# Many98/Crop2Seg

Measured on AMD Instinct MI355X. Metric: train patches/sec (Tx10x128x128) U-TAE, higher is better.
Workload: dtype f32

## Files before the change

### crop2seg_amd/_lib.py

```python
from __future__ import annotations

import ctypes as C
import os
from typing import Optional

HERE = os.path.dirname(os.path.abspath(__file__))
LIB_PATH = os.environ.get("C2S_LIB", os.path.join(HERE, "libc2s_hip.so"))

c_float_p = C.c_void_p
c_int_p = C.c_void_p

PAD_ZEROS, PAD_REFLECT = 0, 1
SRC_F32, SRC_I16, SRC_U16 = 0, 1, 2
NORM_GROUP, NORM_BATCH = 0, 1


class ConvDesc(C.Structure):
    _fields_ = [(n, C.c_int) for n in (
        "N", "C0", "C1", "Hin", "Win", "Cout", "CoutP", "Hout", "Wout", "OutH", "OutW", "KH", "KW", "S",
        "pad_y", "pad_x", "pad_mode", "osy", "osx", "ooy", "oox", "accumulate", "reflect_adjoint")]


class WgradDesc(C.Structure):
    _fields_ = [(n, C.c_int) for n in (
        "N", "C0", "C1", "Hin", "Win", "Cout", "Hout", "Wout", "KH", "KW", "S", "pad_y", "pad_x", "pad_mode",
        "nslices")]


class NormDesc(C.Structure):
    _fields_ = [("N", C.c_int), ("C", C.c_int), ("HW", C.c_int), ("kind", C.c_int), ("groups", C.c_int),
                ("training", C.c_int), ("eps", C.c_float), ("momentum", C.c_float)]


class LtaeDesc(C.Structure):
    _fields_ = [("B", C.c_int), ("T", C.c_int), ("C", C.c_int), ("HW", C.c_int), ("n_head", C.c_int),
                ("d_model", C.c_int), ("eps", C.c_float), ("dropout_p", C.c_float), ("seed", C.c_uint64),
                ("keep", C.c_void_p), ("seed_dev", C.c_void_p), ("keep_bits", C.c_void_p)]


class AggDesc(C.Structure):
    _fields_ = [(n, C.c_int) for n in ("B", "T", "C", "H", "W", "n_head", "h", "w")]


P = C.c_void_p
I = C.c_int
L = C.c_long
F = C.c_float
SZ = C.c_size_t

SIGNATURES = {
    "c2s_abi_version": (I, []),
    "c2s_last_error": (C.c_char_p, []),
    "c2s_init": (I, [I]),
    "c2s_device_cus": (I, []),
    "c2s_pack_weights": (I, [P, P, I, I, I, I, L, L, C.POINTER(I), P]),
    "c2s_pack_job_bytes": (SZ, []),
    "c2s_pack_job_fill": (I, [P, P, P, I, I, I, I, L, L, I, C.POINTER(I), I]),
    "c2s_pack_job_blocks": (I, [I, I, I, I]),
    "c2s_pack_batch": (I, [P, I, I, P]),
    "c2s_conv_igemm": (I, [C.POINTER(ConvDesc), P, P, P, P, P, P, P]),
    "c2s_conv_xpair": (I, [C.POINTER(ConvDesc), P, P, P, P, P, P]),
    "c2s_conv3x3_smallcin_supported": (I, [C.POINTER(ConvDesc)]),
    "c2s_conv3x3_smallcin": (I, [C.POINTER(ConvDesc), P, P, P, P, P, P]),
    "c2s_winograd_packed_floats": (SZ, [I, I]),
    "c2s_pack_weights_winograd": (I, [P, P, I, I, I, L, L, C.POINTER(I), P]),
    "c2s_conv3x3_winograd": (I, [C.POINTER(ConvDesc), P, P, P, P, P, P, P]),
    "c2s_winograd16_packed_floats": (SZ, [I, I]),
    "c2s_pack_weights_winograd16": (I, [P, P, I, I, I, L, L, C.POINTER(I), P]),
    "c2s_conv3x3_winograd16_supported": (I, [C.POINTER(ConvDesc)]),
    "c2s_conv3x3_winograd16": (I, [C.POINTER(ConvDesc), P, P, P, P, P, P, P]),
    "c2s_s2wino_packed_floats": (SZ, [I, I]),
    "c2s_pack_weights_s2wino": (I, [P, P, I, I, I, L, L, C.POINTER(I), P]),
    "c2s_conv4x4s2_winograd_supported": (I, [C.POINTER(ConvDesc)]),
    "c2s_conv4x4s2_winograd": (I, [C.POINTER(ConvDesc), P, P, P, P, P, P]),
    "c2s_s2dgrad_packed_floats": (SZ, [I, I]),
    "c2s_pack_weights_s2dgrad": (I, [P, P, I, I, I, L, L, C.POINTER(I), P]),
    "c2s_conv4x4s2_dgrad_winograd_supported": (I, [C.POINTER(ConvDesc)]),
    "c2s_conv4x4s2_dgrad_winograd": (I, [C.POINTER(ConvDesc), P, P, P, P, P]),
    "c2s_bf16x3_packed_elems": (SZ, [I, I]),
    "c2s_pack_weights_bf16x3": (I, [P, P, P, I, I, I, I, L, L, C.POINTER(I), P]),
    "c2s_conv3x3_bf16x3": (I, [C.POINTER(ConvDesc), P, P, P, P, P, P, P, P]),
    "c2s_bf16x3_set_single_product": (None, [I]),
    "c2s_wgrad_workspace_floats": (SZ, [C.POINTER(WgradDesc)]),
    "c2s_conv_wgrad": (I, [C.POINTER(WgradDesc), P, P, P, P, SZ, P, P]),
    "c2s_wgrad_algorithms": (I, [I, I]),
    "c2s_wgrad_path": (I, [C.POINTER(WgradDesc), C.POINTER(I)]),
    "c2s_wgrad_reduce": (I, [C.POINTER(WgradDesc), P, P, L, L, C.POINTER(I), I, P]),
    "c2s_wgrad_reduce_job_bytes": (SZ, []),
    "c2s_wgrad_reduce_job_blocks": (I, [C.POINTER(WgradDesc)]),
    "c2s_wgrad_reduce_job_fill": (I, [P, C.POINTER(WgradDesc), P, P, L, L, C.POINTER(I), I, I]),
    "c2s_wgrad_reduce_batch": (I, [P, I, I, P]),
    "c2s_dwconv_fwd": (I, [P, P, P, P, I, I, I, I, I, I, I, I, P]),
    "c2s_dwconv_dgrad": (I, [P, P, P, P, I, I, I, I, I, I, I, I, I, P]),
    "c2s_dwconv_wgrad": (I, [P, P, P, P, P, I, I, I, I, I, I, I, I, P]),
    "c2s_norm_workspace_floats": (SZ, [C.POINTER(NormDesc)]),
    "c2s_norm_fwd": (I, [C.POINTER(NormDesc), P, P, P, P, P, P, P, P, P, P, I, P, SZ, P, F, P]),
    "c2s_norm_bwd": (I, [C.POINTER(NormDesc), P, P, P, P, P, I, P, P, P, P, P, SZ, P, P]),
    "c2s_norm_bwd_params": (I, [C.POINTER(NormDesc), P, P, P, P, P, P]),
    "c2s_norm_onepass_sync_bytes": (SZ, [C.POINTER(NormDesc), I]),
    "c2s_norm_fwd_onepass": (I, [C.POINTER(NormDesc), P, P, P, P, P, P, P, P, P, P, I, P, F, P, SZ, P]),
    "c2s_norm_bwd_onepass": (I, [C.POINTER(NormDesc), P, P, P, P, P, I, P, P, P, P, P, SZ, P, P, SZ, P]),
    "c2s_se_workspace_floats": (SZ, [I, I, I]),
    "c2s_channel_bias_add": (I, [P, P, P, I, I, I, P]),
    "c2s_se_fwd": (I, [P, P, P, P, P, P, P, P, I, I, I, F, P, SZ, P]),
    "c2s_se_bwd": (I, [P, P, P, P, P, P, P, P, P, P, I, I, P, I, I, I, P, SZ, P]),
    "c2s_frame_flags": (I, [P, P, I, L, F, P]),
    "c2s_ltae_attn_fwd": (I, [C.POINTER(LtaeDesc)] + [P] * 13 + [P]),
    "c2s_positional_table": (I, [P, P, L, C.c_float, P]),
    "c2s_ltae_fold_fwd": (I, [P] * 9 + [I, I, P]),
    "c2s_ltae_fold_bwd": (I, [P] * 16 + [I, I, I, P, SZ, P]),
    "c2s_ltae_fold_bwd_workspace_floats": (SZ, []),
    "c2s_ltae_pe_table": (I, [I, P, P, F, P, P, P, P, P, I, P]),
    "c2s_ltae_pe_abs_add": (I, [P, P, P, P, P, I, P]),
    "c2s_ltae_pe_abs_bwd": (I, [P, P, P, P, I, P]),
    "c2s_ltae_pe_fwd": (I, [P, P, P, P, P, I, I, I, I, P]),
    "c2s_ltae_pe_gattn": (I, [P, P, P, P, I, I, I, P]),
    "c2s_ltae_pe_bwd": (I, [I] + [P] * 15 + [I, I, I, P]),
    "c2s_ltae_fwd_workspace_floats": (SZ, [C.POINTER(LtaeDesc)]),
    "c2s_ltae_attn_fwd_ws": (I, [C.POINTER(LtaeDesc)] + [P] * 13 + [P, SZ, P]),
    "c2s_ltae_uses_streaming": (I, [C.POINTER(LtaeDesc)]),
    "c2s_ltae_fwd_path": (I, [C.POINTER(LtaeDesc)]),
    "c2s_ltae_attn_optional": (I, [C.POINTER(LtaeDesc)]),
    "c2s_ltae_paths": (I, [C.POINTER(LtaeDesc), I, P, P]),
    "c2s_ltae_bwd_workspace_floats": (SZ, [C.POINTER(LtaeDesc)]),
    "c2s_ltae_attn_bwd": (I, [C.POINTER(LtaeDesc)] + [P] * 22 + [SZ, P]),
    "c2s_dropout_nchw": (I, [P, P, I, I, I, F, C.c_uint64, P, P, P]),
    "c2s_pixel_gn_fwd": (I, [P, P, P, P, P, I, I, I, I, F, P]),
    "c2s_pixel_gn_bwd_workspace_floats": (SZ, [I, I, I]),
    "c2s_pixel_gn_bwd": (I, [P, P, P, P, P, P, P, I, I, I, I, P, SZ, P]),
    "c2s_attn_head_mean": (I, [P, P, I, L, P]),
    "c2s_attn_head_mean_bwd": (I, [P, P, I, L, I, P]),
    "c2s_frame_mean_weights": (I, [P, P, I, I, I, P]),
    "c2s_temporal_aggregate_fwd": (I, [C.POINTER(AggDesc), P, P, P, P, P]),
    "c2s_temporal_aggregate_bwd_workspace_floats": (SZ, [C.POINTER(AggDesc)]),
    "c2s_temporal_aggregate_bwd": (I, [C.POINTER(AggDesc), P, P, P, P, P, I, P, P, SZ, P]),
    "c2s_cross_entropy_workspace_floats": (SZ, [I, I]),
    "c2s_cross_entropy": (I, [P, P, P, P, P, I, I, I, F, C.c_longlong, P, SZ, P]),
    "c2s_metrics_update": (I, [P, P, P, P, P, P, I, I, I, P]),
    "c2s_confusion_add": (I, [P, P, P, L, I, P]),
    "c2s_loss_meter_add": (I, [P, P, P]),
    "c2s_boundary_target": (I, [P, P, I, I, I, P]),
    "c2s_region_relabel": (I, [P, P, I, I, I, I, C.c_longlong, P]),
    "c2s_focal_ce_workspace_floats": (SZ, []),
    "c2s_focal_ce": (I, [P, P, P, P, I, I, I, F, C.c_longlong, I, P, SZ, P]),
    "c2s_focal_ce_ex": (I, [P, P, P, P, P, I, I, I, F, C.c_longlong, I, I, P, SZ, P]),
    "c2s_smooth_ce_workspace_floats": (SZ, []),
    "c2s_smooth_ce": (I, [P, P, P, P, P, P, I, I, I, I, F, C.c_longlong, I, P, SZ, P]),
    "c2s_smooth_ce_ex": (I, [P, P, P, P, P, P, P, I, I, I, I, F, C.c_longlong, I, I, P, SZ, P]),
    "c2s_parcel_seeds": (I, [P, P, P, P, I, I, I, I, I, I, F, P]),
    "c2s_label_components_workspace_bytes": (SZ, [I, I, I]),
    "c2s_label_components": (I, [P, P, P, I, I, I, I, P, SZ, P, P]),
    "c2s_parcel_vote_workspace_bytes": (SZ, [I, I, I]),
    "c2s_parcel_vote": (I, [P, P, P, P, I, I, I, I, I, F, I, P, SZ, P, P]),
    "c2s_collate_series": (I, [P, I, P, P, P, P, P, I, I, I, I, I, C.POINTER(I), C.POINTER(F), C.POINTER(F), F, P]),
    "c2s_collate_series_ndvi": (I, [P, I, P, P, P, P, P, I, I, I, I, I, C.POINTER(I), C.POINTER(F), C.POINTER(F), F, I, I, P]),
    "c2s_softmax_stitch": (I, [P, P, P, I, I, I, I, I, I, I, I, P]),
    "c2s_adam_flat": (I, [P, P, P, P, L, F, F, F, F, I, P, F, P]),
    "c2s_grad_sumsq_workspace_doubles": (SZ, []),
    "c2s_grad_sumsq": (I, [P, P, P, I, L, P, SZ, P, P]),
    "c2s_step_decide": (I, [P, F, F, I, P, P, I, P, P]),
    "c2s_adam_slots": (I, [P, P, P, P, P, P, P, I, L, F, F, F, F, P, P]),
    "c2s_restore_if_skipped": (I, [P, P, L, P, P]),
    "c2s_fill": (I, [P, L, F, P]),
    "c2s_add_inplace": (I, [P, P, L, P]),
}

_LIB: Optional[C.CDLL] = None


class C2SError(RuntimeError):
    pass


def lib() -> C.CDLL:
    global _LIB
    if _LIB is None:
        if not os.path.exists(LIB_PATH):
            raise C2SError(
                f"{LIB_PATH} not found: build it with `python -m crop2seg_amd.build` "
                "(or __graft_entry__.build()); crop2seg_amd has no CPU/PyTorch fallback")
        handle = C.CDLL(LIB_PATH)
        for name, (res, args) in SIGNATURES.items():
            fn = getattr(handle, name)
            fn.restype = res
            fn.argtypes = args
        _LIB = handle
    return _LIB


_INITED = set()


def init_device(index: int) -> None:
    if index in _INITED:
        return
    check(lib().c2s_init(index), "c2s_init")
    _INITED.add(index)


def check(rc: int, what: str) -> None:
    if rc != 0:
        msg = lib().c2s_last_error().decode(errors="replace")
        raise C2SError(f"{what} failed (code {rc}): {msg}")
```

### crop2seg_amd/csrc/conv_igemm.hip

```cpp
#include "common.h"

namespace {

struct ConvParams {
    const float* src0;
    const float* src1;
    const float* wpk;
    const float* bias;
    float* out;
    const int* valid;
    int C0, C1, Hin, Win, Cout, CoutP, Hout, Wout, OutH, OutW;
    int pad_y, pad_x, pad_mode, osy, osx, ooy, oox, accumulate;
    int log2fc, tiles_x;
    int adj, ay_lo, ay_hi, ax_lo, ax_hi;
    int dy_lo, dy_hi, dx_lo, dx_hi;
};

constexpr int cmax(int a, int b) { return a > b ? a : b; }
constexpr int plane_for(int K, int S, int log2fc) {
    return ((8 * (32 >> log2fc) - 1) * S + K) * (((1 << log2fc) - 1) * S + K);
}
constexpr int max_plane(int K, int S) {
    return cmax(cmax(plane_for(K, S, 2), plane_for(K, S, 3)), cmax(plane_for(K, S, 4), plane_for(K, S, 5)));
}

template <int K, int S>
struct Cfg {
    static constexpr int CK = K == 1 ? 16 : (K == 2 ? 8 : (K >= 4 ? 2 : 4));
    static constexpr int NT = K * K;
    static constexpr int MAXE = (CK * max_plane(K, S) + 255) / 256;
};

template <int K, int S, int MF, bool ADJ>
__global__ __launch_bounds__(256) void conv_igemm_kernel(ConvParams p) {
    constexpr int CK = Cfg<K, S>::CK;
    constexpr int NT = Cfg<K, S>::NT;
    constexpr int MAXE = Cfg<K, S>::MAXE;
    constexpr int COT = 32 * MF;
    constexpr int WV = COT / 4;
    constexpr int NWV = NT * CK * WV;
    constexpr int WPT = (NWV + 255) / 256;
    constexpr int NS = NT * (CK / 2);
    extern __shared__ float lds[];

    int bxi = blockIdx.x, n = blockIdx.z;
    {
        const unsigned tot = gridDim.x * gridDim.z;
        if (gridDim.y == 1 && (tot & 7) == 0) {
            const unsigned lin = blockIdx.x + gridDim.x * blockIdx.z;
            const unsigned l2_ = (lin & 7) * (tot >> 3) + (lin >> 3);
            n = (int)(l2_ / gridDim.x);
            bxi = (int)(l2_ - (unsigned)n * gridDim.x);
        }
    }
    if (p.valid != nullptr && p.valid[n] == 0) return;

    const int FC = 1 << p.log2fc, FR = 32 >> p.log2fc;
    const int tile_h = 8 * FR, tile_w = FC;
    const int rows = (tile_h - 1) * S + K, cols = (tile_w - 1) * S + K;
    const int plane = rows * cols;
    float* Xl = lds;
    const int xsz = (CK * plane + 3) & ~3;
    float* Wl = lds + xsz;
    const int BUF = xsz + NT * CK * COT;

    const int tyi = bxi / p.tiles_x, txi = bxi % p.tiles_x;
    const int oy0 = tyi * tile_h, ox0 = txi * tile_w;
    const int co0 = blockIdx.y * COT;
    const int tid = threadIdx.x;
    const int Cin = p.C0 + p.C1;
    const int HWin = p.Hin * p.Win;

    int goff[MAXE];
    const int total = CK * plane;
#pragma unroll
    for (int i = 0; i < MAXE; ++i) {
        const int e = tid + i * 256;
        int off = -1;
        if (e < total) {
            const int c = e / plane;
            const int rem = e - c * plane;
            const int r = rem / cols;
            const int cc = rem - r * cols;
            int gy = oy0 * S - p.pad_y + r;
            int gx = ox0 * S - p.pad_x + cc;
            bool ok;
            if (p.pad_mode == C2S_PAD_REFLECT) {
                ok = gy >= -p.pad_y && gy < p.Hin + p.pad_y && gx >= -p.pad_x && gx < p.Win + p.pad_x;
                gy = reflect_idx(gy, p.Hin);
                gx = reflect_idx(gx, p.Win);
            } else {
                ok = gy >= 0 && gy < p.Hin && gx >= 0 && gx < p.Win;
            }
            if (ok) off = (c * HWin + gy * p.Win + gx) * 4;
        }
        goff[i] = off;
    }

    const int lane = tid & 63, wave = tid >> 6;
    const int li = lane & 31, lk = lane >> 5;
    const int fy = li >> p.log2fc, fx = li & (FC - 1);
    int boff[2];
#pragma unroll
    for (int q = 0; q < 2; ++q) {
        const int f = 2 * wave + q;
        boff[q] = lk * plane + ((f * FR + fy) * S) * cols + fx * S;
    }
    const int aoff = lk * COT + li;

    float mxlo[2] = {0.f, 0.f}, mxhi[2] = {0.f, 0.f}, mylo[2] = {0.f, 0.f}, myhi[2] = {0.f, 0.f};
    if constexpr (ADJ) {
#pragma unroll
        for (int q = 0; q < 2; ++q) {
            const int f = 2 * wave + q;
            const int oy = oy0 + f * FR + fy, ox = ox0 + fx;
            mxlo[q] = ox == p.ax_lo ? 1.f : 0.f;
            mxhi[q] = ox == p.ax_hi ? 1.f : 0.f;
            mylo[q] = oy == p.ay_lo ? 1.f : 0.f;
            myhi[q] = oy == p.ay_hi ? 1.f : 0.f;
        }
    }

    f32x16 acc[MF][2];
#pragma unroll
    for (int m = 0; m < MF; ++m)
#pragma unroll
        for (int q = 0; q < 2; ++q)
#pragma unroll
            for (int r = 0; r < 16; ++r) acc[m][q][r] = 0.f;

    const float* s0n = p.src0 + (size_t)n * p.C0 * HWin;
    const float* s1n = p.src1 != nullptr ? p.src1 + (size_t)n * p.C1 * HWin : nullptr;
    const __amdgpu_buffer_rsrc_t r0 = __builtin_amdgcn_make_buffer_rsrc((void*)s0n, 0, p.C0 * HWin * 4, 0x00020000);
    const __amdgpu_buffer_rsrc_t r1 = __builtin_amdgcn_make_buffer_rsrc((void*)(s1n != nullptr ? s1n : s0n), 0,
                                                                         p.C1 * HWin * 4, 0x00020000);
    const __amdgpu_buffer_rsrc_t rw = __builtin_amdgcn_make_buffer_rsrc((void*)p.wpk, 0, NT * Cin * p.CoutP * 4, 0x00020000);

    float xr[MAXE];
    f32x4 wr[WPT];
    auto prefetch = [&](int cb) {
        const bool first = cb < p.C0;
        const int chan0 = (first ? cb : cb - p.C0) * HWin * 4;
        if (first) {
#pragma unroll
            for (int i = 0; i < MAXE; ++i)
                xr[i] = __builtin_bit_cast(float, __builtin_amdgcn_raw_buffer_load_b32(r0, goff[i] >= 0 ? goff[i] + chan0 : -1, 0, 0));
        } else {
#pragma unroll
            for (int i = 0; i < MAXE; ++i)
                xr[i] = __builtin_bit_cast(float, __builtin_amdgcn_raw_buffer_load_b32(r1, goff[i] >= 0 ? goff[i] + chan0 : -1, 0, 0));
        }
#pragma unroll
        for (int i = 0; i < WPT; ++i) {
            const int e = tid + i * 256;
            const int o4 = e % WV, tc = e / WV;
            const int c = tc % CK, t = tc / CK;
            const bool ok = e < NWV && cb + c < Cin;
            const int off = ok ? (((t * Cin + cb + c) * p.CoutP + co0 + o4 * 4) * 4) : -1;
            wr[i] = __builtin_bit_cast(f32x4, __builtin_amdgcn_raw_buffer_load_b128(rw, off, 0, 0));
        }
    };
    auto commit = [&](int buf) {
        float* Xd = Xl + buf * BUF;
        float* Wd = Wl + buf * BUF;
#pragma unroll
        for (int i = 0; i < MAXE; ++i) {
            const int e = tid + i * 256;
            if (e < total) Xd[e] = xr[i];
        }
#pragma unroll
        for (int i = 0; i < WPT; ++i) {
            const int e = tid + i * 256;
            if (e < NWV) *reinterpret_cast<f32x4*>(Wd + (size_t)e * 4) = wr[i];
        }
    };

    auto load_ops = [&](const float* Xl, const float* Wl, int s_, float (&a)[MF], float (&b)[2]) {
        const int t = s_ / (CK / 2), cp = s_ % (CK / 2);
        const int ky = t / K, kx = t % K;
#pragma unroll
        for (int m = 0; m < MF; ++m) a[m] = Wl[(t * CK + 2 * cp) * COT + aoff + m * 32];
#pragma unroll
        for (int q = 0; q < 2; ++q) {
            const int ad = boff[q] + 2 * cp * plane + ky * cols + kx;
            float v = Xl[ad];
            if constexpr (ADJ) {
                const bool xl = kx == K - 1, xh = kx == 0, yl = ky == K - 1, yh = ky == 0;
                const int dx = xl ? -p.dx_lo : p.dx_hi;
                if (xl || xh) {
                    const float mx = xl ? mxlo[q] : mxhi[q];
                    v = fmaf(mx, Xl[ad + dx], v);
                }
                if (yl || yh) {
                    const float my = yl ? mylo[q] : myhi[q];
                    const int dy = (yl ? -p.dy_lo : p.dy_hi) * cols;
                    v = fmaf(my, Xl[ad + dy], v);
                    if (xl || xh) {
                        const float mx = xl ? mxlo[q] : mxhi[q];
                        v = fmaf(my * mx, Xl[ad + dy + dx], v);
                    }
                }
            }
            b[q] = v;
        }
    };

    constexpr int COMMIT_AT = NS / 2;
    prefetch(0);
    commit(0);
    if (CK < Cin) prefetch(CK);
    __syncthreads();
    int cur = 0;
    for (int cb = 0; cb < Cin; cb += CK, cur ^= 1) {
        const float* Xc = Xl + cur * BUF;
        const float* Wc = Wl + cur * BUF;
        float a[2][MF], b[2][2];
        load_ops(Xc, Wc, 0, a[0], b[0]);
#pragma unroll
        for (int s_ = 0; s_ < NS; ++s_) {
            if (s_ + 1 < NS) load_ops(Xc, Wc, s_ + 1, a[(s_ + 1) & 1], b[(s_ + 1) & 1]);
            __builtin_amdgcn_sched_barrier(0);
#pragma unroll
            for (int m = 0; m < MF; ++m)
#pragma unroll
                for (int q = 0; q < 2; ++q)
                    acc[m][q] = __builtin_amdgcn_mfma_f32_32x32x2f32(a[s_ & 1][m], b[s_ & 1][q], acc[m][q], 0, 0, 0);
            __builtin_amdgcn_sched_barrier(0);
            if (s_ == COMMIT_AT && cb + CK < Cin) {
                commit(cur ^ 1);
                if (cb + 2 * CK < Cin) prefetch(cb + 2 * CK);
                __builtin_amdgcn_sched_barrier(0);
            }
        }
        __syncthreads();
    }

    const size_t outHW = (size_t)p.OutH * p.OutW;
    float* on = p.out + (size_t)n * p.Cout * outHW;
#pragma unroll
    for (int q = 0; q < 2; ++q) {
        const int f = 2 * wave + q;
        const int oy = oy0 + f * FR + fy, ox = ox0 + fx;
        if (oy >= p.Hout || ox >= p.Wout) continue;
        const size_t sp = (size_t)(oy * p.osy + p.ooy) * p.OutW + (ox * p.osx + p.oox);
#pragma unroll
        for (int m = 0; m < MF; ++m) {
#pragma unroll
            for (int r0 = 0; r0 < 16; r0 += 8) {
                float old[8];
                if (p.accumulate) {
#pragma unroll
                    for (int u = 0; u < 8; ++u) {
                        const int r = r0 + u;
                        const int co = co0 + m * 32 + (r & 3) + 8 * (r >> 2) + 4 * lk;
                        old[u] = co < p.Cout ? on[(size_t)co * outHW + sp] : 0.f;
                    }
                }
#pragma unroll
                for (int u = 0; u < 8; ++u) {
                    const int r = r0 + u;
                    const int co = co0 + m * 32 + (r & 3) + 8 * (r >> 2) + 4 * lk;
                    if (co < p.Cout) {
                        float v = acc[m][q][r];
                        if (p.bias != nullptr) v += p.bias[co];
                        if (p.accumulate) v += old[u];
                        on[(size_t)co * outHW + sp] = v;
                    }
                }
            }
        }
    }
}

template <int K, int S, int MF, bool ADJ>
int launch_conv(const ConvParams& p, int N, int tiles, hipStream_t st) {
    constexpr int CK = Cfg<K, S>::CK;
    constexpr int NT = Cfg<K, S>::NT;
    const int FC = 1 << p.log2fc, FR = 32 >> p.log2fc;
    const int rows = (8 * FR - 1) * S + K, cols = (FC - 1) * S + K;
    const size_t lds = 2 * ((((size_t)CK * rows * cols + 3) & ~(size_t)3) + (size_t)NT * CK * 32 * MF) * sizeof(float);
    dim3 grid(tiles, p.CoutP / (32 * MF), N);
    hipLaunchKernelGGL((conv_igemm_kernel<K, S, MF, ADJ>), grid, dim3(256), lds, st, p);
    C2S_CHECK_LAUNCH("conv_igemm");
    return C2S_OK;
}

void init_hook() {
#define C2S_RAISE4(K_, S_)                               \
    C2S_RAISE_LDS((conv_igemm_kernel<K_, S_, 1, false>)); \
    C2S_RAISE_LDS((conv_igemm_kernel<K_, S_, 2, false>));
    C2S_RAISE4(3, 1) C2S_RAISE4(1, 1) C2S_RAISE4(2, 1) C2S_RAISE4(4, 2) C2S_RAISE4(2, 2) C2S_RAISE4(6, 2)
#undef C2S_RAISE4
    C2S_RAISE_LDS((conv_igemm_kernel<3, 1, 1, true>));
    C2S_RAISE_LDS((conv_igemm_kernel<3, 1, 2, true>));
    C2S_RAISE_LDS((conv_igemm_kernel<2, 1, 1, true>));
    C2S_RAISE_LDS((conv_igemm_kernel<2, 1, 2, true>));
}
C2sInitRegistrar registrar(init_hook);

}

extern "C" int c2s_conv_igemm(const c2s_conv_desc* d, const float* src0, const float* src1, const float* wpk,
                              const float* bias, float* out, const int* valid, void* stream) {
    C2S_REQUIRE(d && src0 && wpk && out, "conv_igemm: null pointer");
    C2S_REQUIRE(d->N > 0 && d->C0 > 0 && d->C1 >= 0 && (d->C1 == 0 || src1), "conv_igemm: bad channels");
    C2S_REQUIRE(d->CoutP % 32 == 0 && d->CoutP >= d->Cout && d->Cout > 0, "conv_igemm: CoutP must be a multiple of 32");
    C2S_REQUIRE(d->KH == d->KW, "conv_igemm: square kernels only");
    C2S_REQUIRE(d->C1 == 0 || d->C0 % 16 == 0, "conv_igemm: with two sources C0 must be a multiple of 16");
    C2S_REQUIRE((long)(d->C0 > d->C1 ? d->C0 : d->C1) * d->Hin * d->Win * 4 < (1L << 31), "conv_igemm: frame too large");
    C2S_REQUIRE((long)d->Hin * d->Win < (1 << 20), "conv_igemm: input plane too large");
    C2S_REQUIRE(d->Hout > 0 && d->Wout > 0, "conv_igemm: empty output");
    C2S_REQUIRE((d->Hout - 1) * d->osy + d->ooy < d->OutH && (d->Wout - 1) * d->osx + d->oox < d->OutW,
                "conv_igemm: output placement exceeds the output plane");
    if (d->pad_mode == C2S_PAD_REFLECT)
        C2S_REQUIRE(d->pad_y < d->Hin && d->pad_x < d->Win, "conv_igemm: reflect padding needs pad < size");
    ConvParams p;
    p.src0 = src0; p.src1 = src1; p.wpk = wpk; p.bias = bias; p.out = out; p.valid = valid;
    p.C0 = d->C0; p.C1 = d->C1; p.Hin = d->Hin; p.Win = d->Win; p.Cout = d->Cout; p.CoutP = d->CoutP;
    p.Hout = d->Hout; p.Wout = d->Wout; p.OutH = d->OutH; p.OutW = d->OutW;
    p.pad_y = d->pad_y; p.pad_x = d->pad_x; p.pad_mode = d->pad_mode;
    p.osy = d->osy; p.osx = d->osx; p.ooy = d->ooy; p.oox = d->oox; p.accumulate = d->accumulate;
    p.adj = d->reflect_adjoint;
    p.ay_lo = p.ay_hi = p.ax_lo = p.ax_hi = -1;
    p.dy_lo = p.dy_hi = p.dx_lo = p.dx_hi = d->KH - 1;
    if (d->reflect_adjoint == 2) {
        C2S_REQUIRE(d->pad_mode == C2S_PAD_ZEROS && d->S == 1 && d->KH == 3 && d->pad_y == 1 && d->pad_x == 1 &&
                    d->osy == 2 && d->osx == 2 && d->ooy >= 0 && d->ooy <= 1 && d->oox >= 0 && d->oox <= 1 &&
                    d->Hin == d->Hout && d->Win == d->Wout && d->Hin >= 2 && d->Win >= 2,
                    "conv_igemm: reflect_adjoint 2 applies to the parity launches of the 6x6 stride-2 data gradient");
        p.ay_lo = d->ooy == 0 ? 1 : 0;   p.dy_lo = d->ooy == 0 ? 2 : 1;
        p.ay_hi = d->Hout - 1 - d->ooy;  p.dy_hi = d->ooy == 0 ? 1 : 2;
        p.ax_lo = d->oox == 0 ? 1 : 0;   p.dx_lo = d->oox == 0 ? 2 : 1;
        p.ax_hi = d->Wout - 1 - d->oox;  p.dx_hi = d->oox == 0 ? 1 : 2;
    } else if (d->reflect_adjoint) {
        C2S_REQUIRE(d->pad_mode == C2S_PAD_ZEROS && d->S == 1 && (d->KH == 3 || d->KH == 2),
                    "conv_igemm: reflect_adjoint applies to the zero-padded 3x3 / 2x2-parity data-gradient launches");
        C2S_REQUIRE(d->Hin >= 2 && d->Win >= 2 && d->Hin != 3 && d->Win != 3, "conv_igemm: reflect_adjoint needs planes of 2 or >= 4");
        if (d->KH == 3) {
            C2S_REQUIRE(d->pad_y == 1 && d->pad_x == 1 && d->Hin == d->Hout && d->Win == d->Wout, "conv_igemm: bad 3x3 adjoint geometry");
            p.ay_lo = 1; p.ay_hi = d->Hout - 2;
            p.ax_lo = 1; p.ax_hi = d->Wout - 2;
        } else {
            if (d->pad_y == 0) p.ay_lo = 0; else p.ay_hi = d->Hout - 1;
            if (d->pad_x == 0) p.ax_lo = 0; else p.ax_hi = d->Wout - 1;
        }
    }
    int l2 = 5;
    while (l2 > 2 && (1 << l2) > d->Wout) --l2;
    p.log2fc = l2;
    const int FC = 1 << l2, FR = 32 >> l2;
    p.tiles_x = cdiv(d->Wout, FC);
    const int tiles = p.tiles_x * cdiv(d->Hout, 8 * FR);
    hipStream_t st = (hipStream_t)stream;
    const int cus = c2s_cus();
    const bool wide = d->CoutP % 64 == 0 && (long)tiles * d->N * (d->CoutP / 64) >= 2L * cus;
#define C2S_DISPATCH(K_, S_, A_)                                        \
    if (d->KH == K_ && d->S == S_ && (p.adj != 0) == A_)                \
        return wide ? launch_conv<K_, S_, 2, A_>(p, d->N, tiles, st) : launch_conv<K_, S_, 1, A_>(p, d->N, tiles, st);
    C2S_DISPATCH(3, 1, false)
    C2S_DISPATCH(3, 1, true)
    C2S_DISPATCH(1, 1, false)
    C2S_DISPATCH(2, 1, false)
    C2S_DISPATCH(2, 1, true)
    C2S_DISPATCH(4, 2, false)
    C2S_DISPATCH(2, 2, false)
    C2S_DISPATCH(6, 2, false)
#undef C2S_DISPATCH
    c2s_set_error("conv_igemm: unsupported (K=%d,S=%d)", d->KH, d->S);
    return C2S_EINVAL;
}
```

### include/c2s_hip.h

```cpp
#ifndef C2S_HIP_H
#define C2S_HIP_H

#include <stddef.h>
#include <stdint.h>

#ifdef __cplusplus
extern "C" {
#endif

#define C2S_OK 0
#define C2S_EINVAL (-1)
#define C2S_ELAUNCH (-2)
#define C2S_ENOSPACE (-3)

#define C2S_PAD_ZEROS 0
#define C2S_PAD_REFLECT 1

#define C2S_NORM_GROUP 0
#define C2S_NORM_BATCH 1

int c2s_abi_version(void);
const char* c2s_last_error(void);
int c2s_init(int device);
int c2s_device_cus(void);

int c2s_pack_weights(const float* src, float* wpk, int cin, int cout, int coutP, int ntaps,
                     long stride_o, long stride_c, const int* host_tap_off, void* stream);
size_t c2s_pack_job_bytes(void);
int c2s_pack_job_fill(void* host_record, const float* src, float* dst, int cin, int cout, int coutP, int ntaps,
                      long stride_o, long stride_c, int winograd, const int* host_tap_off, int block_start);
int c2s_pack_job_blocks(int cin, int coutP, int ntaps, int winograd);
int c2s_pack_batch(const void* device_table, int njobs, int total_blocks, void* stream);


typedef struct c2s_conv_desc {
    int N, C0, C1;
    int Hin, Win;
    int Cout, CoutP;
    int Hout, Wout;
    int OutH, OutW;
    int KH, KW, S;
    int pad_y, pad_x;
    int pad_mode;
    int osy, osx, ooy, oox;
    int accumulate;
    int reflect_adjoint;
} c2s_conv_desc;

int c2s_conv_igemm(const c2s_conv_desc* d, const float* src0, const float* src1, const float* wpk,
                   const float* bias, float* out, const int* valid, void* stream);

int c2s_conv3x3_smallcin_supported(const c2s_conv_desc* d);
int c2s_conv3x3_smallcin(const c2s_conv_desc* d, const float* src, const float* wpk, const float* bias, float* out,
                         const int* valid, void* stream);

int c2s_conv_xpair(const c2s_conv_desc* d, const float* src, const float* wpk, const float* bias, float* out,
                   const int* valid, void* stream);

size_t c2s_winograd_packed_floats(int cin, int coutP);
int c2s_pack_weights_winograd(const float* src, float* upk, int cin, int cout, int coutP, long stride_o, long stride_c,
                              const int* host_tap_off, void* stream);
int c2s_conv3x3_winograd(const c2s_conv_desc* d, const float* src0, const float* src1, const float* upk,
                         const float* bias, float* out, const int* valid, void* stream);

size_t c2s_winograd16_packed_floats(int cin, int coutP);
int c2s_pack_weights_winograd16(const float* src, float* upk, int cin, int cout, int coutP, long stride_o, long stride_c,
                                const int* host_tap_off, void* stream);
int c2s_conv3x3_winograd16_supported(const c2s_conv_desc* d);
int c2s_conv3x3_winograd16(const c2s_conv_desc* d, const float* src0, const float* src1, const float* upk,
                           const float* bias, float* out, const int* valid, void* stream);

size_t c2s_s2wino_packed_floats(int cin, int coutP);
int c2s_pack_weights_s2wino(const float* src, float* upk, int cin, int cout, int coutP, long stride_o, long stride_c,
                            const int* host_tap_off, void* stream);
int c2s_conv4x4s2_winograd_supported(const c2s_conv_desc* d);
int c2s_conv4x4s2_winograd(const c2s_conv_desc* d, const float* src, const float* upk, const float* bias, float* out,
                           const int* valid, void* stream);

size_t c2s_s2dgrad_packed_floats(int kc, int csP);
int c2s_pack_weights_s2dgrad(const float* src, float* upk, int kc, int cs, int csP, long stride_c, long stride_k,
                             const int* host_tap_off, void* stream);
int c2s_conv4x4s2_dgrad_winograd_supported(const c2s_conv_desc* d);
int c2s_conv4x4s2_dgrad_winograd(const c2s_conv_desc* d, const float* gy, const float* upk, float* gx, const int* valid,
                                 void* stream);

size_t c2s_bf16x3_packed_elems(int cin, int coutP);
int c2s_pack_weights_bf16x3(const float* src, void* whi, void* wlo, int cin, int cout, int coutP, int ntaps,
                            long stride_o, long stride_c, const int* host_tap_off, void* stream);
int c2s_conv3x3_bf16x3(const c2s_conv_desc* d, const float* src0, const float* src1, const void* whi,
                       const void* wlo, const float* bias, float* out, const int* valid, void* stream);
void c2s_bf16x3_set_single_product(int on);

typedef struct c2s_wgrad_desc {
    int N, C0, C1, Hin, Win;
    int Cout;
    int Hout, Wout;
    int KH, KW, S, pad_y, pad_x, pad_mode;
    int nslices;
} c2s_wgrad_desc;

size_t c2s_wgrad_workspace_floats(const c2s_wgrad_desc* d);
int c2s_conv_wgrad(const c2s_wgrad_desc* d, const float* src0, const float* src1, const float* gout,
                   float* slabs, size_t slab_floats, const int* valid, void* stream);
int c2s_wgrad_algorithms(int winograd_3x3, int winograd_4x4s2);
int c2s_wgrad_path(const c2s_wgrad_desc* d, int* family);
int c2s_wgrad_reduce(const c2s_wgrad_desc* d, const float* slabs, float* dst, long stride_o, long stride_c,
                     const int* host_tap_off, int accumulate, void* stream);
size_t c2s_wgrad_reduce_job_bytes(void);
int c2s_wgrad_reduce_job_blocks(const c2s_wgrad_desc* d);
int c2s_wgrad_reduce_job_fill(void* host_record, const c2s_wgrad_desc* d, const float* slabs, float* dst, long stride_o,
                              long stride_c, const int* host_tap_off, int accumulate, int block_start);
int c2s_wgrad_reduce_batch(const void* device_table, int njobs, int total_blocks, void* stream);

int c2s_dwconv_fwd(const float* in, const float* w, float* out, const int* valid, int N, int C, int Hin, int Win,
                   int K, int S, int pad, int pad_mode, void* stream);
int c2s_dwconv_dgrad(const float* gout, const float* w, float* gin, const int* valid, int N, int C, int Hin, int Win,
                     int K, int S, int pad, int pad_mode, int accumulate, void* stream);
int c2s_dwconv_wgrad(const float* in, const float* gout, float* partial, float* gw, const int* valid, int N, int C,
                     int Hin, int Win, int K, int S, int pad, int pad_mode, void* stream);

typedef struct c2s_norm_desc {
    int N, C, HW;
    int kind;
    int groups;
    int training;
    float eps, momentum;
} c2s_norm_desc;

size_t c2s_norm_workspace_floats(const c2s_norm_desc* d);
int c2s_norm_fwd(const c2s_norm_desc* d, const float* x, const float* gamma, const float* beta,
                 float* running_mean, float* running_var, long long* num_batches_tracked, float* group_stats, float* row_ab,
                 const float* residual, float* y, int relu, float* workspace, size_t ws_floats, const int* valid,
                 float pad_value, void* stream);
int c2s_norm_bwd(const c2s_norm_desc* d, const float* x, const float* g, const float* gamma,
                 const float* group_stats, const float* row_ab, int relu, float* gx, float* dgamma,
                 float* dbeta, float* dbias, float* workspace, size_t ws_floats, const int* valid, void* stream);
int c2s_norm_bwd_params(const c2s_norm_desc* d, const float* workspace, float* dgamma, float* dbeta, float* dbias,
                        const int* valid, void* stream);

size_t c2s_norm_onepass_sync_bytes(const c2s_norm_desc* d, int has_valid);
int c2s_norm_fwd_onepass(const c2s_norm_desc* d, const float* x, const float* gamma, const float* beta,
                         float* running_mean, float* running_var, long long* num_batches_tracked, float* group_stats,
                         float* row_ab, const float* residual, float* y, int relu, const int* valid, float pad_value,
                         void* sync, size_t sync_bytes, void* stream);
int c2s_norm_bwd_onepass(const c2s_norm_desc* d, const float* x, const float* g, const float* gamma,
                         const float* group_stats, const float* row_ab, int relu, float* gx, float* dgamma, float* dbeta,
                         float* dbias, float* workspace, size_t ws_floats, const int* valid, void* sync,
                         size_t sync_bytes, void* stream);

size_t c2s_se_workspace_floats(int N, int C, int HW);
int c2s_channel_bias_add(float* x, const float* bias, const int* valid, int N, int C, int HW, void* stream);
int c2s_se_fwd(const float* x, const float* W1, const float* W2, float* pooled, float* hidden, float* scale, float* y,
               const int* valid, int N, int C, int HW, float pad_value, float* workspace, size_t ws_floats, void* stream);
int c2s_se_bwd(const float* x, const float* g, const float* W1, const float* W2, const float* pooled, const float* hidden,
               const float* scale, float* gx, float* gW1, float* gW2, int acc_w1, int acc_w2, const int* valid, int N, int C,
               int HW, float* workspace, size_t ws_floats, void* stream);

int c2s_frame_flags(const float* x, int* valid, int N, long frame_elems, float pad_value, void* stream);

typedef struct c2s_ltae_desc {
    int B, T, C, HW;
    int n_head, d_model;
    float eps;
    float dropout_p;
    uint64_t seed;
    const float* keep;
    const uint64_t* seed_dev;
    uint64_t* keep_bits;
} c2s_ltae_desc;

int c2s_ltae_attn_fwd(const c2s_ltae_desc* d, const float* x, const float* gamma, const float* beta,
                      const float* U, const float* s0, const float* Wc, const float* bc, const float* pe,
                      const int* valid, float* attn, float* attn_pre, float* emb, float* stats, void* stream);
size_t c2s_ltae_fwd_workspace_floats(const c2s_ltae_desc* d);
int c2s_ltae_attn_fwd_ws(const c2s_ltae_desc* d, const float* x, const float* gamma, const float* beta,
                         const float* U, const float* s0, const float* Wc, const float* bc, const float* pe,
                         const int* valid, float* attn, float* attn_pre, float* emb, float* stats,
                         float* workspace, size_t ws_floats, void* stream);
int c2s_ltae_uses_streaming(const c2s_ltae_desc* d);
int c2s_ltae_fwd_path(const c2s_ltae_desc* d);
int c2s_ltae_attn_optional(const c2s_ltae_desc* d);
int c2s_ltae_paths(const c2s_ltae_desc* d, int with_emb, int* fwd, int* bwd);
size_t c2s_ltae_bwd_workspace_floats(const c2s_ltae_desc* d);
int c2s_ltae_attn_bwd(const c2s_ltae_desc* d, const float* x, const float* gamma, const float* beta,
                      const float* U, const float* s0, const float* Wc, const float* bc, const float* pe,
                      const int* valid, const float* attn, const float* attn_pre, const float* stats,
                      const float* g_emb, const float* g_attn, float* gx, float* gU, float* gs0, float* gWc,
                      float* gbc, float* ggamma, float* gbeta, float* workspace, size_t ws_floats, void* stream);

int c2s_positional_table(const long long* dates, float* pe, long n, float period, void* stream);
int c2s_ltae_fold_fwd(const float* Q, const float* Wk, const float* bk, const float* Wc, const float* bc, const float* pe,
                      float* U, float* s0, float* qwk, int BT, int C, void* stream);
int c2s_ltae_fold_bwd(const float* Q, const float* Wk, const float* bk, const float* Wc, const float* bc, const float* pe,
                      const float* qwk, const float* gU, const float* gs0, const float* gWc_attn, const float* gbc_attn,
                      float* gQ, float* gWk, float* gbk, float* gWc, float* gbc, int BT, int C, int acc_mask,
                      float* workspace, size_t ws_floats, void* stream);
size_t c2s_ltae_fold_bwd_workspace_floats(void);

int c2s_ltae_pe_table(int mode, const long long* dates0, const long long* dates1, float period, const float* W, const float* b,
                      float* pe256, float* sin256, int* bad_days, int BT, void* stream);
int c2s_ltae_pe_abs_add(const long long* dates1, const float* W2, const float* b2, float* pe256, int* bad_days, int BT,
                        void* stream);
int c2s_ltae_pe_abs_bwd(const long long* dates1, const float* g_pe, float* gW2, float* gb2, int BT, void* stream);
int c2s_ltae_pe_fwd(const float* qwk, const float* pe256, const float* attn, float* s0, float* emb, int B, int T, int HW,
                    int phase, void* stream);
int c2s_ltae_pe_gattn(const float* g_emb, const float* pe256, const float* g_attn_in, float* g_attn_out, int B, int T, int HW,
                      void* stream);
int c2s_ltae_pe_bwd(int mode, const long long* dates0, const long long* dates1, const float* Q, const float* Wk,
                    const float* qwk, const float* pe256, const float* sin256, const float* attn, const float* g_emb,
                    const float* gs0, float* g_pe, float* gWk, float* gQ, float* gW, float* gb, int B, int T, int HW,
                    void* stream);

int c2s_dropout_nchw(const float* x, float* y, int B, int C, int HW, float p, uint64_t seed, const uint64_t* seed_dev,
                     const float* keep, void* stream);
int c2s_pixel_gn_fwd(const float* x, const float* gamma, const float* beta, float* y, float* stats, int B, int C,
                     int HW, int groups, float eps, void* stream);
size_t c2s_pixel_gn_bwd_workspace_floats(int B, int C, int HW);
int c2s_pixel_gn_bwd(const float* x, const float* gy, const float* gamma, const float* stats, float* gx,
                     float* dgamma, float* dbeta, int B, int C, int HW, int groups, float* workspace,
                     size_t ws_floats, void* stream);

typedef struct c2s_agg_desc {
    int B, T, C, H, W;
    int n_head, h, w;
} c2s_agg_desc;

int c2s_attn_head_mean(const float* attn, float* v, int n_head, long n, void* stream);
int c2s_attn_head_mean_bwd(const float* gv, float* gattn, int n_head, long n, int accumulate, void* stream);
int c2s_frame_mean_weights(const int* valid, float* v, int n_head, int B, int T, void* stream);
int c2s_temporal_aggregate_fwd(const c2s_agg_desc* d, const float* x, const float* attn, const int* valid,
                               float* out, void* stream);
size_t c2s_temporal_aggregate_bwd_workspace_floats(const c2s_agg_desc* d);
int c2s_temporal_aggregate_bwd(const c2s_agg_desc* d, const float* x, const float* attn, const int* valid,
                               const float* gout, float* gx, int gx_accumulate, float* gattn,
                               float* workspace, size_t ws_floats, void* stream);

size_t c2s_cross_entropy_workspace_floats(int B, int HW);
int c2s_cross_entropy(const float* logits, const int64_t* target, const float* class_w, float* loss,
                      float* glogits, int B, int K, int HW, float label_smoothing, long long ignore_index,
                      float* workspace, size_t ws_floats, void* stream);
int c2s_adam_flat(float* p, const float* g, float* m, float* v, long n, float lr, float b1, float b2, float eps,
                  int step, const int* step_dev, float grad_scale, void* stream);

#define C2S_GUARD_STATUS_BYTES 32
size_t c2s_grad_sumsq_workspace_doubles(void);
int c2s_grad_sumsq(const float* g, const long* slots, const int* mask, int nslots, long total, double* workspace,
                   size_t ws_doubles, void* status, void* stream);
int c2s_step_decide(void* status, float max_grad_norm, float grad_scale, int skip_nonfinite, const int* mask,
                    int* slot_steps, int nslots, int* skip_count, void* stream);
int c2s_adam_slots(float* p, const float* g, float* m, float* v, const long* slots, const int* mask,
                   const int* slot_steps, int nslots, long total, float lr, float b1, float b2, float eps,
                   const void* status, void* stream);
int c2s_restore_if_skipped(float* dst, const float* saved, long n, const void* status, void* stream);

int c2s_metrics_update(const float* logits, const long long* target, long long* conf, long long* conf_top2,
                       long long* pred, long long* pred_top2, int B, int K, int HW, void* stream);
int c2s_confusion_add(const long long* pred, const long long* target, long long* conf, long n, int K, void* stream);
int c2s_loss_meter_add(const float* loss, double* acc, void* stream);
int c2s_boundary_target(const long long* y, long long* y_b, int B, int H, int W, void* stream);
int c2s_region_relabel(const long long* y, long long* y_out, int B, int H, int W, int keep_boundary, long long ignore_label,
                       void* stream);
size_t c2s_focal_ce_workspace_floats(void);
int c2s_focal_ce(const float* logits, const long long* target, float* loss, float* glogits, int B, int K, int HW,
                 float gamma, long long ignore_index, int accumulate_loss, float* workspace, size_t ws_floats,
                 void* stream);
int c2s_focal_ce_ex(const float* logits, const long long* target, const float* class_w, float* loss, float* glogits, int B,
                    int K, int HW, float gamma, long long ignore_index, int size_average, int accumulate_loss,
                    float* workspace, size_t ws_floats, void* stream);
size_t c2s_smooth_ce_workspace_floats(void);
int c2s_smooth_ce(const float* logits, const long long* target, const float* class_w, const float* bg_distrib, float* loss,
                  float* glogits, int B, int K, int H, int W, float label_smoothing, long long bg_index, int accumulate_loss,
                  float* workspace, size_t ws_floats, void* stream);
int c2s_smooth_ce_ex(const float* logits, const long long* target, const float* class_w, const float* bg_distrib, float* loss,
                     float* glogits, float* pixel_loss, int B, int K, int H, int W, float label_smoothing, long long bg_index,
                     int reduction, int accumulate_loss, float* workspace, size_t ws_floats, void* stream);

int c2s_parcel_seeds(const float* scores, const float* boundary_scores, unsigned char* mask, long long* t1, int B, int K,
                     int H, int W, int from_logits, int boundary_code, float second_threshold, void* stream);
size_t c2s_label_components_workspace_bytes(int B, int H, int W);
int c2s_label_components(const unsigned char* mask, int* labels, int* count, int B, int H, int W, int min_size,
                         void* workspace, size_t ws_bytes, int* error, void* stream);
size_t c2s_parcel_vote_workspace_bytes(int B, int cap, int K);
int c2s_parcel_vote(const long long* pred, const int* labels, long long* out, int* parcel_class, int B, int H, int W, int K,
                    int cap, float bg_share, int outside, void* workspace, size_t ws_bytes, int* error, void* stream);

#define C2S_SRC_F32 0
#define C2S_SRC_I16 1
#define C2S_SRC_U16 2
int c2s_collate_series(const void* src, int src_dtype, const long long* offsets, const long long* src_dates, float* x,
                       long long* dates, int* valid, int B, int T, int C, int Cs, int HW,
                       const int* host_channel_order, const float* host_mean, const float* host_std, float pad_value,
                       void* stream);
int c2s_collate_series_ndvi(const void* src, int src_dtype, const long long* offsets, const long long* src_dates, float* x,
                            long long* dates, int* valid, int B, int T, int C, int Cs, int HW, const int* host_channel_order,
                            const float* host_mean, const float* host_std, float pad_value, int ndvi_a, int ndvi_b,
                            void* stream);
int c2s_softmax_stitch(const float* logits, float* proba, long long* top1, int first_patch, int npatch, int K, int ph,
                       int pw, int grid_w, int out_h, int out_w, void* stream);

int c2s_fill(float* p, long n, float v, void* stream);
int c2s_add_inplace(float* dst, const float* src, long n, void* stream);

#ifdef __cplusplus
}
#endif
#endif
```

Measured before the change: 369.6.

## Split igemm conv spatial tiles into smaller workgroups when grid underfills CUs

Adds split variants of the implicit-GEMM conv kernel that cover half or a quarter of the spatial tile rows. The SP=4 variant uses 128 threads, and both split variants use one fragment per wave and a deeper operand prefetch. A heuristic picks the split when the default grid would have fewer than two workgroups per CU, and an environment variable can force a choice. The aim is better occupancy on small late-layer convolutions. The cost is more redundant halo loads and weight staging per output, and more kernel instantiations.

```diff
diff --git a/crop2seg_amd/_lib.py b/crop2seg_amd/_lib.py
--- a/crop2seg_amd/_lib.py
+++ b/crop2seg_amd/_lib.py
@@ -59,6 +59,7 @@
     "c2s_pack_job_blocks": (I, [I, I, I, I]),
     "c2s_pack_batch": (I, [P, I, I, P]),
     "c2s_conv_igemm": (I, [C.POINTER(ConvDesc), P, P, P, P, P, P, P]),
+    "c2s_conv_igemm_split": (I, [C.POINTER(ConvDesc), I]),
     "c2s_conv_xpair": (I, [C.POINTER(ConvDesc), P, P, P, P, P, P]),
     "c2s_conv3x3_smallcin_supported": (I, [C.POINTER(ConvDesc)]),
     "c2s_conv3x3_smallcin": (I, [C.POINTER(ConvDesc), P, P, P, P, P, P]),
diff --git a/crop2seg_amd/csrc/conv_igemm.hip b/crop2seg_amd/csrc/conv_igemm.hip
--- a/crop2seg_amd/csrc/conv_igemm.hip
+++ b/crop2seg_amd/csrc/conv_igemm.hip
@@ -17,29 +17,35 @@
 };
 
 constexpr int cmax(int a, int b) { return a > b ? a : b; }
-constexpr int plane_for(int K, int S, int log2fc) {
-    return ((8 * (32 >> log2fc) - 1) * S + K) * (((1 << log2fc) - 1) * S + K);
-}
-constexpr int max_plane(int K, int S) {
-    return cmax(cmax(plane_for(K, S, 2), plane_for(K, S, 3)), cmax(plane_for(K, S, 4), plane_for(K, S, 5)));
-}
-
-template <int K, int S>
+constexpr int plane_for(int K, int S, int log2fc, int NF) {
+    return ((NF * (32 >> log2fc) - 1) * S + K) * (((1 << log2fc) - 1) * S + K);
+}
+constexpr int max_plane(int K, int S, int NF) {
+    return cmax(cmax(plane_for(K, S, 2, NF), plane_for(K, S, 3, NF)), cmax(plane_for(K, S, 4, NF), plane_for(K, S, 5, NF)));
+}
+
+template <int K, int S, int SP = 1>
 struct Cfg {
     static constexpr int CK = K == 1 ? 16 : (K == 2 ? 8 : (K >= 4 ? 2 : 4));
     static constexpr int NT = K * K;
-    static constexpr int MAXE = (CK * max_plane(K, S) + 255) / 256;
+    static constexpr int NTHR = SP == 4 ? 128 : 256;
+    static constexpr int MAXE = (CK * max_plane(K, S, 8 / SP) + NTHR - 1) / NTHR;
 };
 
-template <int K, int S, int MF, bool ADJ>
-__global__ __launch_bounds__(256) void conv_igemm_kernel(ConvParams p) {
-    constexpr int CK = Cfg<K, S>::CK;
-    constexpr int NT = Cfg<K, S>::NT;
-    constexpr int MAXE = Cfg<K, S>::MAXE;
+template <int K, int S, int MF, bool ADJ, int SP = 1>
+__global__ __launch_bounds__((Cfg<K, S, SP>::NTHR)) void conv_igemm_kernel(ConvParams p) {
+    static_assert(SP == 1 || ((SP == 2 || SP == 4) && MF == 1), "the split tiles exist for 32-channel tiles");
+    constexpr int CK = Cfg<K, S, SP>::CK;
+    constexpr int NT = Cfg<K, S, SP>::NT;
+    constexpr int MAXE = Cfg<K, S, SP>::MAXE;
+    constexpr int NTHR = Cfg<K, S, SP>::NTHR;
+    constexpr int NF = 8 / SP;
+    constexpr int NQ = SP == 1 ? 2 : 1;
+    constexpr int LA = SP == 1 ? 1 : 2;
     constexpr int COT = 32 * MF;
     constexpr int WV = COT / 4;
     constexpr int NWV = NT * CK * WV;
-    constexpr int WPT = (NWV + 255) / 256;
+    constexpr int WPT = (NWV + NTHR - 1) / NTHR;
     constexpr int NS = NT * (CK / 2);
     extern __shared__ float lds[];
 
@@ -56,7 +62,7 @@
     if (p.valid != nullptr && p.valid[n] == 0) return;
 
     const int FC = 1 << p.log2fc, FR = 32 >> p.log2fc;
-    const int tile_h = 8 * FR, tile_w = FC;
+    const int tile_h = NF * FR, tile_w = FC;
     const int rows = (tile_h - 1) * S + K, cols = (tile_w - 1) * S + K;
     const int plane = rows * cols;
     float* Xl = lds;
@@ -75,7 +81,7 @@
     const int total = CK * plane;
 #pragma unroll
     for (int i = 0; i < MAXE; ++i) {
-        const int e = tid + i * 256;
+        const int e = tid + i * NTHR;
         int off = -1;
         if (e < total) {
             const int c = e / plane;
@@ -100,19 +106,19 @@
     const int lane = tid & 63, wave = tid >> 6;
     const int li = lane & 31, lk = lane >> 5;
     const int fy = li >> p.log2fc, fx = li & (FC - 1);
-    int boff[2];
-#pragma unroll
-    for (int q = 0; q < 2; ++q) {
-        const int f = 2 * wave + q;
+    int boff[NQ];
+#pragma unroll
+    for (int q = 0; q < NQ; ++q) {
+        const int f = NQ * wave + q;
         boff[q] = lk * plane + ((f * FR + fy) * S) * cols + fx * S;
     }
     const int aoff = lk * COT + li;
 
-    float mxlo[2] = {0.f, 0.f}, mxhi[2] = {0.f, 0.f}, mylo[2] = {0.f, 0.f}, myhi[2] = {0.f, 0.f};
+    float mxlo[NQ] = {}, mxhi[NQ] = {}, mylo[NQ] = {}, myhi[NQ] = {};
     if constexpr (ADJ) {
 #pragma unroll
-        for (int q = 0; q < 2; ++q) {
-            const int f = 2 * wave + q;
+        for (int q = 0; q < NQ; ++q) {
+            const int f = NQ * wave + q;
             const int oy = oy0 + f * FR + fy, ox = ox0 + fx;
             mxlo[q] = ox == p.ax_lo ? 1.f : 0.f;
             mxhi[q] = ox == p.ax_hi ? 1.f : 0.f;
@@ -121,11 +127,11 @@
         }
     }
 
-    f32x16 acc[MF][2];
+    f32x16 acc[MF][NQ];
 #pragma unroll
     for (int m = 0; m < MF; ++m)
 #pragma unroll
-        for (int q = 0; q < 2; ++q)
+        for (int q = 0; q < NQ; ++q)
 #pragma unroll
             for (int r = 0; r < 16; ++r) acc[m][q][r] = 0.f;
 
@@ -152,7 +158,7 @@
         }
 #pragma unroll
         for (int i = 0; i < WPT; ++i) {
-            const int e = tid + i * 256;
+            const int e = tid + i * NTHR;
             const int o4 = e % WV, tc = e / WV;
             const int c = tc % CK, t = tc / CK;
             const bool ok = e < NWV && cb + c < Cin;
@@ -165,23 +171,23 @@
         float* Wd = Wl + buf * BUF;
 #pragma unroll
         for (int i = 0; i < MAXE; ++i) {
-            const int e = tid + i * 256;
+            const int e = tid + i * NTHR;
             if (e < total) Xd[e] = xr[i];
         }
 #pragma unroll
         for (int i = 0; i < WPT; ++i) {
-            const int e = tid + i * 256;
+            const int e = tid + i * NTHR;
             if (e < NWV) *reinterpret_cast<f32x4*>(Wd + (size_t)e * 4) = wr[i];
         }
     };
 
-    auto load_ops = [&](const float* Xl, const float* Wl, int s_, float (&a)[MF], float (&b)[2]) {
+    auto load_ops = [&](const float* Xl, const float* Wl, int s_, float (&a)[MF], float (&b)[NQ]) {
         const int t = s_ / (CK / 2), cp = s_ % (CK / 2);
         const int ky = t / K, kx = t % K;
 #pragma unroll
         for (int m = 0; m < MF; ++m) a[m] = Wl[(t * CK + 2 * cp) * COT + aoff + m * 32];
 #pragma unroll
-        for (int q = 0; q < 2; ++q) {
+        for (int q = 0; q < NQ; ++q) {
             const int ad = boff[q] + 2 * cp * plane + ky * cols + kx;
             float v = Xl[ad];
             if constexpr (ADJ) {
@@ -214,17 +220,18 @@
     for (int cb = 0; cb < Cin; cb += CK, cur ^= 1) {
         const float* Xc = Xl + cur * BUF;
         const float* Wc = Wl + cur * BUF;
-        float a[2][MF], b[2][2];
-        load_ops(Xc, Wc, 0, a[0], b[0]);
+        float a[LA + 1][MF], b[LA + 1][NQ];
+#pragma unroll
+        for (int s_ = 0; s_ < LA; ++s_) load_ops(Xc, Wc, s_, a[s_], b[s_]);
 #pragma unroll
         for (int s_ = 0; s_ < NS; ++s_) {
-            if (s_ + 1 < NS) load_ops(Xc, Wc, s_ + 1, a[(s_ + 1) & 1], b[(s_ + 1) & 1]);
+            if (s_ + LA < NS) load_ops(Xc, Wc, s_ + LA, a[(s_ + LA) % (LA + 1)], b[(s_ + LA) % (LA + 1)]);
             __builtin_amdgcn_sched_barrier(0);
 #pragma unroll
             for (int m = 0; m < MF; ++m)
 #pragma unroll
-                for (int q = 0; q < 2; ++q)
-                    acc[m][q] = __builtin_amdgcn_mfma_f32_32x32x2f32(a[s_ & 1][m], b[s_ & 1][q], acc[m][q], 0, 0, 0);
+                for (int q = 0; q < NQ; ++q)
+                    acc[m][q] = __builtin_amdgcn_mfma_f32_32x32x2f32(a[s_ % (LA + 1)][m], b[s_ % (LA + 1)][q], acc[m][q], 0, 0, 0);
             __builtin_amdgcn_sched_barrier(0);
             if (s_ == COMMIT_AT && cb + CK < Cin) {
                 commit(cur ^ 1);
@@ -238,8 +245,8 @@
     const size_t outHW = (size_t)p.OutH * p.OutW;
     float* on = p.out + (size_t)n * p.Cout * outHW;
 #pragma unroll
-    for (int q = 0; q < 2; ++q) {
-        const int f = 2 * wave + q;
+    for (int q = 0; q < NQ; ++q) {
+        const int f = NQ * wave + q;
         const int oy = oy0 + f * FR + fy, ox = ox0 + fx;
         if (oy >= p.Hout || ox >= p.Wout) continue;
         const size_t sp = (size_t)(oy * p.osy + p.ooy) * p.OutW + (ox * p.osx + p.oox);
@@ -272,15 +279,15 @@
     }
 }
 
-template <int K, int S, int MF, bool ADJ>
+template <int K, int S, int MF, bool ADJ, int SP = 1>
 int launch_conv(const ConvParams& p, int N, int tiles, hipStream_t st) {
-    constexpr int CK = Cfg<K, S>::CK;
-    constexpr int NT = Cfg<K, S>::NT;
+    constexpr int CK = Cfg<K, S, SP>::CK;
+    constexpr int NT = Cfg<K, S, SP>::NT;
     const int FC = 1 << p.log2fc, FR = 32 >> p.log2fc;
-    const int rows = (8 * FR - 1) * S + K, cols = (FC - 1) * S + K;
+    const int rows = ((8 / SP) * FR - 1) * S + K, cols = (FC - 1) * S + K;
     const size_t lds = 2 * ((((size_t)CK * rows * cols + 3) & ~(size_t)3) + (size_t)NT * CK * 32 * MF) * sizeof(float);
     dim3 grid(tiles, p.CoutP / (32 * MF), N);
-    hipLaunchKernelGGL((conv_igemm_kernel<K, S, MF, ADJ>), grid, dim3(256), lds, st, p);
+    hipLaunchKernelGGL((conv_igemm_kernel<K, S, MF, ADJ, SP>), grid, dim3(Cfg<K, S, SP>::NTHR), lds, st, p);
     C2S_CHECK_LAUNCH("conv_igemm");
     return C2S_OK;
 }
@@ -295,9 +302,37 @@
     C2S_RAISE_LDS((conv_igemm_kernel<3, 1, 2, true>));
     C2S_RAISE_LDS((conv_igemm_kernel<2, 1, 1, true>));
     C2S_RAISE_LDS((conv_igemm_kernel<2, 1, 2, true>));
+#define C2S_RAISE_SP(K_, S_, A_)                              \
+    C2S_RAISE_LDS((conv_igemm_kernel<K_, S_, 1, A_, 2>));     \
+    C2S_RAISE_LDS((conv_igemm_kernel<K_, S_, 1, A_, 4>));
+    C2S_RAISE_SP(3, 1, false) C2S_RAISE_SP(3, 1, true) C2S_RAISE_SP(1, 1, false) C2S_RAISE_SP(2, 1, false)
+    C2S_RAISE_SP(2, 1, true) C2S_RAISE_SP(4, 2, false) C2S_RAISE_SP(2, 2, false) C2S_RAISE_SP(6, 2, false)
+#undef C2S_RAISE_SP
 }
 C2sInitRegistrar registrar(init_hook);
 
+int frag_log2(const c2s_conv_desc* d) {
+    int l2 = 5;
+    while (l2 > 2 && (1 << l2) > d->Wout) --l2;
+    return l2;
+}
+long split_wgs(const c2s_conv_desc* d, int sp) {
+    const int l2 = frag_log2(d);
+    return (long)cdiv(d->Wout, 1 << l2) * cdiv(d->Hout, (8 / sp) * (32 >> l2)) * d->N * (d->CoutP / 32);
+}
+int forced_split() {
+    const char* e = getenv("C2S_IGEMM_SPLIT");
+    if (e == nullptr || e[0] == 0 || e[1] != 0) return 0;
+    return e[0] == '1' ? 1 : (e[0] == '2' ? 2 : (e[0] == '4' ? 4 : 0));
+}
+
+}
+
+extern "C" int c2s_conv_igemm_split(const c2s_conv_desc* d, int cus) {
+    if (d == nullptr || d->N <= 0 || d->C0 <= 0 || d->C1 < 0 || d->CoutP < 32 || d->Hout <= 0 || d->Wout <= 0 || d->KH <= 0) return 1;
+    if (cus <= 0) cus = c2s_cus();
+    if (split_wgs(d, 1) >= 2L * cus) return 1;
+    return split_wgs(d, 2) >= 2L * cus ? 2 : 4;
 }
 
 extern "C" int c2s_conv_igemm(const c2s_conv_desc* d, const float* src0, const float* src1, const float* wpk,
@@ -345,18 +380,22 @@
             if (d->pad_x == 0) p.ax_lo = 0; else p.ax_hi = d->Wout - 1;
         }
     }
-    int l2 = 5;
-    while (l2 > 2 && (1 << l2) > d->Wout) --l2;
+    const int l2 = frag_log2(d);
     p.log2fc = l2;
     const int FC = 1 << l2, FR = 32 >> l2;
     p.tiles_x = cdiv(d->Wout, FC);
-    const int tiles = p.tiles_x * cdiv(d->Hout, 8 * FR);
     hipStream_t st = (hipStream_t)stream;
     const int cus = c2s_cus();
-    const bool wide = d->CoutP % 64 == 0 && (long)tiles * d->N * (d->CoutP / 64) >= 2L * cus;
-#define C2S_DISPATCH(K_, S_, A_)                                        \
-    if (d->KH == K_ && d->S == S_ && (p.adj != 0) == A_)                \
-        return wide ? launch_conv<K_, S_, 2, A_>(p, d->N, tiles, st) : launch_conv<K_, S_, 1, A_>(p, d->N, tiles, st);
+    const int forced = forced_split();
+    const int sp = forced ? forced : c2s_conv_igemm_split(d, cus);
+    const int tiles = p.tiles_x * cdiv(d->Hout, (8 / sp) * FR);
+    const bool wide = sp == 1 && d->CoutP % 64 == 0 && (long)tiles * d->N * (d->CoutP / 64) >= 2L * cus;
+#define C2S_DISPATCH(K_, S_, A_)                                                   \
+    if (d->KH == K_ && d->S == S_ && (p.adj != 0) == A_) {                         \
+        if (sp == 2) return launch_conv<K_, S_, 1, A_, 2>(p, d->N, tiles, st);     \
+        if (sp == 4) return launch_conv<K_, S_, 1, A_, 4>(p, d->N, tiles, st);     \
+        return wide ? launch_conv<K_, S_, 2, A_>(p, d->N, tiles, st) : launch_conv<K_, S_, 1, A_>(p, d->N, tiles, st); \
+    }
     C2S_DISPATCH(3, 1, false)
     C2S_DISPATCH(3, 1, true)
     C2S_DISPATCH(1, 1, false)
diff --git a/include/c2s_hip.h b/include/c2s_hip.h
--- a/include/c2s_hip.h
+++ b/include/c2s_hip.h
@@ -49,6 +49,7 @@
 
 int c2s_conv_igemm(const c2s_conv_desc* d, const float* src0, const float* src1, const float* wpk,
                    const float* bias, float* out, const int* valid, void* stream);
+int c2s_conv_igemm_split(const c2s_conv_desc* d, int cus);
 
 int c2s_conv3x3_smallcin_supported(const c2s_conv_desc* d);
 int c2s_conv3x3_smallcin(const c2s_conv_desc* d, const float* src, const float* wpk, const float* bias, float* out,
```

Result: faster. 376.2, median of 6 (+1.8%).
